# linebender/piet-metal

Measured on AMD Instinct MI355X. Metric: Mpixels/s, Ghostscript Tiger 3840x2160 (fills+strokes): W*H / t_frame, higher is better.
Workload: dtype f32 geometry + f16 accumulators (as the reference)

## Files before the change

### piet_metal_amd/csrc/pm_bin_rows.h

```cpp
#pragma once
#include "pm_kernels_common.h"
#include <pm_params.h>
#include "pm_frame_row.h"

namespace pm {


namespace {

#define PM_PU(field) ParamU32<offsetof(FrameParams, field)>(PR)
#define PM_PP(field) ParamPtr<decltype(FrameParams::field), offsetof(FrameParams, field)>(PR)

}

constexpr uint32_t kCtStride = kStripTiles + 1;
#ifndef PM_BIN_SURV_LDS
#define PM_BIN_SURV_LDS 512
#endif
constexpr uint32_t kSurvLds = PM_BIN_SURV_LDS;
constexpr uint32_t kSupCPL = 2;
constexpr uint32_t kChunkCPL = 4;
static_assert(kSuperChunks == 2 * kChunkCPL && kSupCPL <= kCtStride, "two lanes per surviving super; the list fits in s_ct");
__device__ __forceinline__ float HalfWidthOf(uint32_t aux0) { return 0.5f * __uint_as_float(aux0) + 0.5f; }

// ... 60 lines not shown
    const ParamRegs PR = LoadParams(P);
    const uint32_t tid = threadIdx.x;
    uint4 srd_e = make_uint4(0u, 0u, 0u, 0u);
    if constexpr (kEntry) {
        srd_e = E->sr_desc[blockIdx.x];
        uint2 bb_e = make_uint2(0u, 0u);
        uint32_t it_e = 0;
        if (!E->use_row_lists && tid < E->n_band_items) {
            bb_e = E->band_bbox[tid];
            it_e = E->band_item != nullptr ? E->band_item[tid] : tid;
        }
#pragma unroll
        for (uint32_t u = 0; u < 256u / kBinThreads; ++u)
            L.s_lut[tid + u * kBinThreads] = E->lut_srgb2lin[tid + u * kBinThreads] | (E->lut_unorm2h[tid + u * kBinThreads] << 16);
        L.s_ct[tid] = bb_e.x;
        L.s_ct[kBinThreads + tid] = bb_e.y;
        L.s_ct[2 * kBinThreads + tid] = it_e;
        srd_e = Scalar4(srd_e);
    }
    const bool bin_wt = kOne || PM_PU(bin_wt) != 0u;
    auto put_quad = [&](uint4 *q, const uint4 v) {
        if (bin_wt) StoreWT16(q, v);
        else *q = v;
    };
    const uint32_t lane = LaneId();
    const uint32_t wave = kW == 1 ? 0u : tid >> 6;
    if (blockIdx.x == 0) {
        for (uint32_t k = tid; k < kTicketParts; k += kBinThreads) PM_PP(ctr_next)->ticket[k].count = 0;
        for (uint32_t k = tid; k < kFifos; k += kBinThreads) {
            PM_PP(ctr_next)->fifo[k].tail = 0;
            PM_PP(ctr_next)->fifo[k].head = 0;
        }
        for (uint32_t k = tid; k < kFifoShards; k += kBinThreads) PM_PP(ctr_next)->done_part[k].count = 0;
    }
    if (blockIdx.x == 0 && tid == 0) {
#pragma unroll
        for (uint32_t k = 0; k < kArenaShards; ++k) {
            PM_PP(ctr_next)->ptcl[k].top = 0;
            PM_PP(ctr_next)->ptcl[k].bin_dwords = 0;
        }
#pragma unroll
        for (uint32_t k = 0; k < kClasses; ++k) PM_PP(ctr_next)->cls[k].count = 0;
        PM_PP(ctr_next)->overflow = 0;
        PM_PP(ctr_next)->done_top.parts = 0;
        PM_PP(ctr_next)->done_top.done = 0;
    }
    for (uint32_t rix = blockIdx.x, rix_next = 0; rix < PM_PU(n_sr_active); rix = rix_next) {
    if (rix != blockIdx.x) LdsBarrier();
    const bool first_row = kEntry && rix == blockIdx.x;
    uint4 srd = srd_e;
    if (!first_row) srd = PM_PP(sr_desc)[rix];
    uint32_t n_band = PM_PU(n_band_items);
    const uint2 *band_bbox = PM_PP(band_bbox);
    const uint32_t *band_item = PM_PP(band_item);
    uint2 bb_next = make_uint2(0u, 0u);
    uint32_t it_next = 0;
    if (PM_PU(use_row_lists)) {
        const uint2 srl = PM_PP(sr_list)[rix];
        const uint32_t lo = __builtin_amdgcn_readfirstlane(srl.x);
        n_band = __builtin_amdgcn_readfirstlane(srl.y);
        band_bbox = PM_PP(row_bbox) + lo;
        band_item = PM_PP(row_item) + lo;
    }
    if (first_row && !PM_PU(use_row_lists)) {
        bb_next = make_uint2(L.s_ct[tid], L.s_ct[kBinThreads + tid]);
        it_next = L.s_ct[2 * kBinThreads + tid];
    } else if (tid < n_band) {
        bb_next = band_bbox[tid];
        it_next = band_item != nullptr ? band_item[tid] : tid;
    }
    if constexpr (kOne) rix_next = __builtin_amdgcn_readfirstlane(PM_PP(sr_next_one)[rix]);
    else rix_next = PM_PU(bin_no_chains) ? 0u : __builtin_amdgcn_readfirstlane(srd.w);
    if (rix_next == 0) rix_next = 0xffffffffu;
    const bool last_row = rix_next == 0xffffffffu;
    auto one_keep = [&](uint32_t n_heavy, uint32_t n_queued) -> uint32_t { return last_row ? OneLaunchKeep(n_heavy, n_queued) : 0u; };
    uint32_t lut_word[256 / kBinThreads] = {};
    if constexpr (!kEntry) {
#pragma unroll
        for (uint32_t u = 0; u < 256u / kBinThreads; ++u) lut_word[u] = PM_PP(lut_srgb2lin)[tid + u * kBinThreads] | (PM_PP(lut_unorm2h)[tid + u * kBinThreads] << 16);
    }
    const uint32_t srx = __builtin_amdgcn_readfirstlane(srd.x);
    const uint32_t strip = srx & 0xffu, row_rel = srx >> 16;
    const uint32_t t_beg = (srx >> 8) & 15u, t_cnt = ((srx >> 12) & 15u) + 1u;
    const uint32_t run_mask = ((1u << t_cnt) - 1u) << t_beg;
    const uint32_t sr = row_rel * PM_PU(strips_x) + strip;
    const uint32_t shard = rix % kArenaShards;
    const uint32_t shard_quads = PM_PU(tarena_cap) / kArenaShards;
    const uint32_t shard_base = shard * shard_quads;
    const uint32_t ty = PM_PU(row0) + row_rel;
    const int sx0 = static_cast<int>(strip * kGroupW);
    const int y0 = static_cast<int>(ty * kTileH);
    const int sy0 = y0 & ~static_cast<int>(kGroupH - 1);
    auto uniform_f = [](int v) { return __uint_as_float(static_cast<uint32_t>(__builtin_amdgcn_readfirstlane(static_cast<int>(__float_as_uint(static_cast<float>(v)))))); };
    const float fsx0 = uniform_f(sx0 + static_cast<int>(t_beg * kTileW)), fsx1 = uniform_f(sx0 + static_cast<int>((t_beg + t_cnt) * kTileW));
    const float fstrip0 = uniform_f(sx0), fstrip1 = uniform_f(sx0 + static_cast<int>(kGroupW));
    const float fy0 = uniform_f(y0), fy1 = uniform_f(y0 + static_cast<int>(kTileH));
    const float fsy0 = uniform_f(sy0), fsy1 = uniform_f(sy0 + static_cast<int>(kGroupH));

    auto stamp = [&](uint32_t k) {
        if (kProfile) {
            if constexpr (kProfile) {
                if (tid == 0) L.s_stamp[k] = static_cast<uint32_t>(wall_clock64());
            }
        }
    };
    bool prof_first = true;
    uint32_t prof_chunks = 0;
    if constexpr (kProfile) {
        if (tid < 14) L.s_stamp[tid] = 0;
    }
    stamp(0);
    if (tid < kStripTiles) {
        L.s_est[tid] = 0;
        L.s_last_kept[tid] = 0;
        L.s_last_solid[tid] = 0;
        L.s_solid_rgba[tid] = 0;
        L.s_head_q[tid] = 0;
        L.s_head_n[tid] = 0;
        L.s_prev_q[tid] = 0;
    }
    if (tid == 0) L.s_alloc[1] = 0;
// ... 34 lines not shown
        const uint32_t heavy_classes = PM_PU(split_mode) ? PM_PU(n_heavy_classes) : 0u;
        ForClasses([&](auto kc) {
            constexpr uint32_t k = decltype(kc)::value;
            const uint32_t mk = static_cast<uint32_t>(__ballot(is_queued && cls == k));
            if (cls == k) my_mask = mk;
            if constexpr (kOne) {
                const uint32_t nk = static_cast<uint32_t>(__popc(mk));
                if (cls > k) before += nk;
                if (k < heavy_classes) n_heavy += nk;
                n_queued += nk;
            } else {
                WriteLane<k>(lane_cnt, static_cast<uint32_t>(__popc(mk)));
            }
        });
        const uint32_t slots = is_queued ? ((3u * est + 1u) * kCmdQuadsNum + kCmdQuadsDen - 1u) / kCmdQuadsDen : 0u;
        const uint32_t slots_incl = WaveInclusiveScan(slots);
        TailState ts;
        ts.qtotal = WaveLast(slots_incl);
        ts.list_off = slots_incl - slots;
        ts.packed = (is_queued ? 1u : 0u) | (cls << 1) | (static_cast<uint32_t>(__popc(my_mask & ((1u << Opaque(lane)) - 1u))) << 4);
        ts.pos = before + (ts.packed >> 4);
        ts.n_heavy = n_heavy;
        ts.n_queued = n_queued;
        ts.qres = 0;
        if (ts.qtotal) {
            if constexpr (kOne) {
                const uint32_t n_keep = one_keep(n_heavy, n_queued);
                const uint32_t give_heavy = n_heavy - (n_heavy ? n_keep : 0u);
                const uint32_t give_light = n_queued - n_heavy - (n_heavy ? 0u : n_keep);
                const uint32_t give = lane == 0u ? give_heavy : give_light;
                Fifo *const ff = &PM_PP(ctr_cur)->fifo[lane == 0u ? 0u : 1u + (blockIdx.x & (kFifoShards - 1u))];
                if (lane < 2u && give) ts.qres = atomicAdd(&ff->tail, give);
            } else {
                if (lane < kClasses && lane_cnt) ts.qres = atomicAdd(&PM_PP(ctr_cur)->cls[lane].count, lane_cnt);
            }
            if (lane == kClasses) ts.qres = AtomicAddOneLane(&PM_PP(ctr_cur)->ptcl[shard].top, ts.qtotal);
        }
        const uint32_t tile = row_rel * PM_PU(tiles_x) + strip * kStripTiles + Opaque(lane);
        const uint32_t state = is_queued ? 0u : (is_solid ? L.s_solid_rgba[tl] : 0xffffffffu);
        if constexpr (!kOne) {
            if (lane < kStripTiles) L.s_solid_rgba[tl] = tile_lane ? state : 0u;
        }
        if (tile_lane) {
            if (bin_wt) StoreWT4(PM_PP(tile_state) + tile, state);
            else PM_PP(tile_state)[tile] = state;
        }
        if constexpr (kOne) {
            if (last_row) {
                if (lane < kStripTiles) R->state[tl] = tile_lane ? state : 0u;
                if (lane == 0u) R->striprow = sr;
            } else {
                const uint32_t st = static_cast<uint32_t>(__shfl(static_cast<int>(tile_lane ? state : 0u), static_cast<int>(lane >> 2)));
                const uint32_t px = strip * kGroupW + lane * 4u;
                if (st != 0u && px < PM_PU(width)) {
                    const uint32_t col = StoreOrder(st, PM_PU(fb_bgra));
                    uint8_t *const base = PM_PP(fb) + static_cast<size_t>(row_rel * kTileH) * PM_PU(fb_stride) + static_cast<size_t>(px) * 4;
                    const uint32_t rows_here = min(kTileH, PM_PU(height) - min(PM_PU(height), ty * kTileH));
                    const bool vec = px + 4u <= PM_PU(width) && PM_PU(fb_vec16) != 0u;
                    for (uint32_t rr = 0; rr < rows_here; ++rr) {
                        uint8_t *dst = base + static_cast<size_t>(rr) * PM_PU(fb_stride);
                        if (vec) *reinterpret_cast<uint4 *>(dst) = make_uint4(col, col, col, col);
                        else
                            for (uint32_t k = 0; k < 4u && px + k < PM_PU(width); ++k) reinterpret_cast<uint32_t *>(dst)[k] = col;
                    }
                }
            }
        }
// ... 8 lines not shown
        }
        if (!ts.qtotal) return;
        const uint32_t cls = (ts.packed >> 1) & 7u;
        const uint32_t used = static_cast<uint32_t>(__builtin_amdgcn_readlane(static_cast<int>(ts.qres), kClasses)) + 1u;
        const uint32_t base = shard_base + used;
        const uint32_t q_base = static_cast<uint32_t>(__shfl(static_cast<int>(ts.qres), static_cast<int>(cls)));
        const bool fits = used + ts.qtotal <= shard_quads && used + ts.qtotal >= used && L.s_alloc[1] == 0u;
        if (!fits && lane == 0) {
            PM_PP(ctr_cur)->overflow = 1;
            *PM_PP(host_overflow) = 1;
        }
        if (ts.packed & 1u) {
            const uint32_t ol = Opaque(lane);
            const uint32_t tile = row_rel * PM_PU(tiles_x) + strip * kStripTiles + ol;
            const uint32_t list_slot = fits ? base + ts.list_off : 0xffffffffu;
            PM_PP(tile_ptcl)[tile] = list_slot;
            uint4 entry = make_uint4((strip * kStripTiles + ol) | (row_rel << 16), list_slot, L.s_head_q[ol], L.s_head_n[ol]);
            if constexpr (kOne) {
                if (!fits) entry.w |= 1u;
                const uint32_t n_keep = one_keep(ts.n_heavy, ts.n_queued);
                const uint32_t h_base = static_cast<uint32_t>(__builtin_amdgcn_readlane(static_cast<int>(ts.qres), 0));
                const uint32_t l_base = static_cast<uint32_t>(__builtin_amdgcn_readlane(static_cast<int>(ts.qres), 1));
                const uint32_t cap = PM_PU(fifo_cap);
                if (ts.pos < n_keep) {
                    R->entry[ts.pos] = entry;
                } else if (ts.pos < ts.n_heavy) {
                    const uint32_t ix = h_base + ts.pos - n_keep;
                    if (ix < cap) StoreWT16(PM_PP(fifo) + ix, entry);
                } else {
                    const uint32_t ix = l_base + ts.pos - (ts.n_heavy ? ts.n_heavy : n_keep);
                    if (ix < cap) StoreWT16(PM_PP(fifo) + static_cast<size_t>(1u + (blockIdx.x & (kFifoShards - 1u))) * cap + ix, entry);
                }
            } else {
                put_quad(PM_PP(queue) + (cls * PM_PU(queue_cap) + q_base + (ts.packed >> 4)), entry);
            }
        }
    };

    uint32_t ncand = 0;
    if (region_end - cursor == PM_PU(sr_empty_dwords)) n_band = 0;
    if constexpr (!kEntry) {
#pragma unroll
        for (uint32_t u = 0; u < 256u / kBinThreads; ++u) L.s_lut[tid + u * kBinThreads] = lut_word[u];
    }
    for (uint32_t ib = 0;; ib += kBatch) {
        const bool more = ib < n_band;
        const uint32_t j = ib + tid;
        bool cand = false;
        uint32_t mask = 0;
        const uint2 bb = bb_next;
        const uint32_t i = it_next;
        if (j + kBatch < n_band) {
            bb_next = band_bbox[j + kBatch];
            it_next = band_item != nullptr ? band_item[j + kBatch] : j + kBatch;
        }
        if (more && tid < kBatch && j < n_band) {
            const int bx = static_cast<int>(bb.x & 0xffffu), by = static_cast<int>(bb.x >> 16);
            const int bz = static_cast<int>(bb.y & 0xffffu), bw = static_cast<int>(bb.y >> 16);
            cand = bz >= sx0 && bx < sx0 + static_cast<int>(kGroupW) && bw >= y0 && by < y0 + static_cast<int>(kTileH);
            if (cand) {
                const int t_lo = (bx > sx0) ? ((bx - sx0) >> 4) : 0;
                int t_hi = (bz - sx0) >> 4;
                if (t_hi > 15) t_hi = 15;
                mask = ((2u << t_hi) - 1u) & ~((1u << t_lo) - 1u) & run_mask;
                cand = mask != 0u;
            }
        }
// ... 669 lines not shown
```

### piet_metal_amd/csrc/pm_coarse.hip

```cpp
#include "pm_kernels_common.h"
#include "pm_coarse_tile.h"

namespace pm {


template <bool kCapture>
__global__ __launch_bounds__(kThreads, PM_COARSE_WPS) void pm_coarse_kernel(FrameParams P) {
    __shared__ CoarseLds s_lds[kWaves];
    CoarseLds &L = s_lds[WaveId()];

    const uint32_t lane = LaneId();
    const uint64_t lanes_below = (1ull << lane) - 1ull;
    uint32_t cls_end[kClasses];
    {
        uint32_t run = 0;
#pragma unroll
        for (uint32_t k = 0; k < kClasses; ++k) {
            run += P.ctr_cur->cls[k].count;
            cls_end[k] = run;
        }
    }
    const uint32_t n_total = cls_end[kClasses - 1];

    const uint32_t wave_global = blockIdx.x * kWaves + (WaveId());
    const uint32_t n_waves = gridDim.x * kWaves;

    for (uint32_t pass = 0; pass * n_waves < n_total; ++pass) {
        const uint32_t slot = pass * n_waves + ((pass & 1u) ? (n_waves - 1u - wave_global) : wave_global);
        if (slot >= n_total) continue;
        uint32_t qix = slot;
#pragma unroll
        for (uint32_t k = 1; k < kClasses; ++k)
            if (slot >= cls_end[k - 1]) qix = k * P.queue_cap + (slot - cls_end[k - 1]);
        const uint4 qe = Scalar4(P.queue[qix]);
        CoarseTile<kCapture>(P, L, qe, lane, lanes_below);
        WaveSync();
    }
}


void LaunchCoarse(const FrameParams &p, uint32_t grid, bool capture, hipStream_t stream, hipEvent_t t0, hipEvent_t t1) {
    if (capture)
        PM_LAUNCH(pm_coarse_kernel<true>, dim3(grid), dim3(kThreads), stream, t0, t1, p);
    else
        PM_LAUNCH(pm_coarse_kernel<false>, dim3(grid), dim3(kThreads), stream, t0, t1, p);
}

}
```

### piet_metal_amd/csrc/pm_context.hip

```cpp
#include <hip/hip_runtime.h>

#include <algorithm>
#include <chrono>
#include <cmath>
#include <cstdio>
#include <cstdlib>
#include <cstring>
#include <new>
#include <string>
#include <vector>

#include "../../include/piet_metal_amd.h"
#include "pm_device.h"
#include "pm_flatten.h"
#include "pm_hit_test.h"
#include "pm_layout.h"

namespace {

thread_local std::string g_last_error;

void SetError(const std::string &s) { g_last_error = s; }

int HipFail(hipError_t e, const char *what) {
// ... 64 lines not shown
            l->lin2srgb[h] = 0;
            continue;
        }
        float y;
        if (x < thr) {
            y = HalfBitsToFloat(RoundHalf(k * x));
        } else {
            const float p = HalfBitsToFloat(HalfBitsFromDouble(std::pow(static_cast<double>(x), ex)));
            const float sp = HalfBitsToFloat(RoundHalf(s * p));
            y = HalfBitsToFloat(RoundHalf(sp - o));
        }
        const float cl = std::fmin(std::fmax(y, 0.0f), 1.0f);
        l->lin2srgb[h] = static_cast<uint8_t>(std::rintf(cl * 255.0f));
    }
}

}


namespace {
constexpr int kMaxSlots = 16;
constexpr int kDefaultFrameStreams = 4;

int EnvInt(const char *name, int dflt, int lo, int hi) {
    const char *v = std::getenv(name);
    if (!v || !*v) return dflt;
    return std::max(lo, std::min(hi, std::atoi(v)));
}
}

struct FrameSlot {
    uint8_t *d_fb = nullptr;
    size_t fb_cap = 0;
    size_t tables_cap = 0;
    uint32_t *d_arena = nullptr;
    uint32_t arena_cap = 0;
    uint4 *d_queue = nullptr;
    uint32_t *d_tile_state = nullptr;
    uint32_t *d_tile_ptcl = nullptr;
    uint32_t *d_tile_ncmd = nullptr;
    uint4 *d_ptcl = nullptr;
    uint32_t ptcl_cap = 0;
    uint2 *d_row_bbox = nullptr;
    uint32_t *d_row_item = nullptr;
    uint64_t row_cap = 0;
    uint32_t state_epoch = 0;
    uint32_t vp_epoch = 0;
    pm::Counters *d_ctr = nullptr;
    uint32_t *h_overflow = nullptr;
    uint32_t *d_overflow = nullptr;
    uint4 *d_fifo = nullptr;
    uint32_t fifo_cap = 0;
    uint32_t parity = 0;
    hipEvent_t ev_done = nullptr;
    bool in_flight = false;
    bool needs_check = false;
    pm::FrameParams params{};
    hipStream_t frame_stream = nullptr;
    bool user_stream = false;
};

struct pm_ctx {
    int device = 0;
    hipStream_t stream = nullptr;
    std::vector<hipStream_t> streams;
    bool fold_clear = true;
// ... 113 lines not shown
    uint32_t query_keep = 0;
    bool idle_seen = false;
    uint32_t query_every = 8;
    int last_slot = -1;

    pm::FlattenCache flatten_cache;
    bool scene_from_paths = false;

    hipEvent_t ev_scene = nullptr;
    hipEvent_t ev_hit = nullptr;
    hipStream_t hit_stream = nullptr;
    bool hit_pending = false;
    uint8_t *d_hit = nullptr;
    size_t hit_cap = 0;

    float t_flatten_ms = 0, t_index_ms = 0, t_arena_ms = 0;
    uint32_t plans_made = 0;

    uint32_t *d_lut_srgb2lin = nullptr;
    uint32_t *d_lut_unorm2h = nullptr;
    uint8_t *d_lut_lin2srgb = nullptr;
};

namespace {

struct WallTimer {
    std::chrono::steady_clock::time_point t0 = std::chrono::steady_clock::now();
    float ms() const { return std::chrono::duration<float, std::milli>(std::chrono::steady_clock::now() - t0).count(); }
};

uint32_t BandRows(const pm_ctx *c) { return c->row1 - c->row0; }
size_t BandTiles(const pm_ctx *c) { return std::max<size_t>(static_cast<size_t>(BandRows(c)) * c->tiles_x, 1); }

int SyncAll(pm_ctx *c) {
    for (hipStream_t q : c->streams) PM_TRY(hipStreamSynchronize(q));
    for (auto &s : c->slot) {
        if (s.in_flight && s.user_stream) PM_TRY(hipEventSynchronize(s.ev_done));
        s.in_flight = false;
    }
    if (c->hit_pending) PM_TRY(hipEventSynchronize(c->ev_hit));
    c->hit_pending = false;
    return PM_OK;
}

void FreeSlotViewport(FrameSlot *s) {
    if (s->d_fb) (void)hipFree(s->d_fb);
    if (s->d_queue) (void)hipFree(s->d_queue);
    if (s->d_fifo) (void)hipFree(s->d_fifo);
    s->d_fifo = nullptr;
    s->fifo_cap = 0;
    s->d_fb = nullptr;
    s->d_queue = nullptr;
    s->fb_cap = s->tables_cap = 0;
    s->d_tile_state = s->d_tile_ptcl = s->d_tile_ncmd = nullptr;
    s->state_epoch = 0;
}

void FreeViewport(pm_ctx *c) {
    for (auto &s : c->slot) {
        FreeSlotViewport(&s);
        s.in_flight = false;
        s.needs_check = false;
    }
    c->last_slot = -1;
}

int AllocSlotViewport(pm_ctx *c, FrameSlot *s) {
    if (s->d_fb && s->vp_epoch == c->vp_epoch) return PM_OK;
    const size_t tiles = BandTiles(c);
    const size_t tables = std::max<size_t>(tiles, 4);
    const size_t fb_want = std::max<size_t>(c->fb_bytes, 16);
    hipError_t e = hipSuccess;
    if (s->d_fb && s->d_queue && s->fb_cap >= fb_want && s->tables_cap >= tables) {
        if (s->d_fifo) (void)hipFree(s->d_fifo);
        s->d_fifo = nullptr;
        s->fifo_cap = 0;
    } else {
        FreeSlotViewport(s);
        e = hipMalloc(&s->d_fb, fb_want);
        if (e == hipSuccess) e = hipMalloc(&s->d_queue, pm::kClasses * tables * sizeof(uint4) + 3 * tables * sizeof(uint32_t));
        if (e == hipSuccess) {
            s->fb_cap = fb_want;
            s->tables_cap = tables;
        }
    }
    s->vp_epoch = c->vp_epoch;
    if (e == hipSuccess) {
        s->d_tile_state = reinterpret_cast<uint32_t *>(s->d_queue + pm::kClasses * tables);
        s->d_tile_ptcl = s->d_tile_state + tables;
        s->d_tile_ncmd = s->d_tile_ptcl + tables;
    }
    s->state_epoch = 0;
    if (e != hipSuccess) {
        if (s->d_fb) (void)hipFree(s->d_fb);
        if (s->d_queue) (void)hipFree(s->d_queue);
        s->d_fb = nullptr;
        s->d_queue = nullptr;
        s->fb_cap = s->tables_cap = 0;
        s->d_tile_state = s->d_tile_ptcl = s->d_tile_ncmd = nullptr;
        return HipFail(e, "hipMalloc(frame slot viewport buffers)");
    }
    return PM_OK;
}

int AllocViewport(pm_ctx *c) {
    c->vp_epoch += 1;
    for (auto &s : c->slot) {
        s.in_flight = false;
        s.needs_check = false;
        if (s.h_overflow) s.h_overflow[2] = 0;
    }
    c->last_slot = -1;
    const uint32_t rows = BandRows(c);
    c->fb_stride = static_cast<size_t>(c->width) * 4;
    c->fb_bytes = c->fb_stride * static_cast<size_t>(rows) * pm::kTileH;
    const int r0 = AllocSlotViewport(c, &c->slot[0]);
    if (r0 != PM_OK) return r0;
    c->arena_dirty = true;
    c->plan_reusable = false;
    c->fb_slots.clear();
    c->fb_applied = false;
    return PM_OK;
}

int ValidateScene(const uint8_t *meta, size_t meta_len, size_t scene_bytes, uint32_t *n_items_out) {
    if (scene_bytes < 8 || meta_len < 8) return PM_ERR_SCENE;
    uint32_t n, items_ix;
    std::memcpy(&n, meta, 4);
    std::memcpy(&items_ix, meta + 4, 4);
    const uint64_t bbox_end = 8ull + 8ull * n;
    const uint64_t items_end = static_cast<uint64_t>(items_ix) + 32ull * n;
// ... 458 lines not shown
    if (r != PM_OK) return r;
    const float t_plan = tm.ms();
    r = EnsureSlotBuffers(c, s);
    if (r != PM_OK) return r;
    if (tm.ms() > 0.05f && std::getenv("PM_HOST_TIMING")) std::fprintf(stderr, "BuildParams: plan %.3f slot buffers %.3f ms (arena %u dwords, tile arena %llu quads)\n", t_plan, tm.ms() - t_plan, c->arena_cap, static_cast<unsigned long long>(c->ptcl_want));
    if (!fb) fb = s->d_fb;
    std::memset(p, 0, sizeof(*p));
    p->scene = c->d_scene;
    p->scene_bytes = static_cast<uint32_t>(c->scene_bytes);
    p->n_items = c->n_items;
    p->items_ix = c->dev_items_ix;
    p->bbox_ix = c->dev_bbox_ix;
    p->width = c->width;
    p->height = c->height;
    p->tiles_x = c->tiles_x;
    p->tiles_y = c->tiles_y;
    p->row0 = c->row0;
    p->row1 = c->row1;
    p->strips_x = c->strips_x;
    p->fb = fb;
    p->fb_stride = static_cast<uint32_t>(stride);
    p->fb_vec16 = ((reinterpret_cast<uintptr_t>(fb) & 15u) == 0 && (stride & 15u) == 0) ? 1u : 0u;
    p->fb_bgra = c->target_fmt == PM_FMT_BGRA8 ? 1u : 0u;
    p->arena = s->d_arena;
    p->arena_cap = s->arena_cap;
    p->sr_desc = c->d_sr_desc;
    p->sr_list = c->d_sr_list;
    p->n_sr_active = c->n_sr_active;
    p->sr_slots = c->d_sr_slots;
    p->bin_prio_slots = c->bin_prio_slots;
    p->bin_grid = c->bin_grid;
    p->sr_empty_dwords = c->sr_empty_dwords;
    p->queue = s->d_queue;
    p->queue_cap = static_cast<uint32_t>(BandTiles(c));
    p->tile_state = s->d_tile_state;
    p->tarena = s->d_ptcl;
    p->tarena_cap = s->ptcl_cap;
    p->tile_ptcl = s->d_tile_ptcl;
    p->tile_ncmd = s->d_tile_ncmd;
    p->ctr_cur = s->d_ctr + s->parity;
    p->ctr_next = s->d_ctr + (s->parity ^ 1u);
    p->host_overflow = s->d_overflow;
    p->host_fail = s->d_overflow + 1;
    p->host_dense = s->d_overflow + 2;
    p->fine_dense = 0;
    p->fifo = s->d_fifo;
    p->fifo_cap = s->fifo_cap;
    p->one_launch = 0;
    p->sr_next_one = c->d_sr_next_one;
    p->one_grid_rows = c->one_grid_rows;
    p->idle_sr = c->d_idle_sr;
    p->n_idle_sr = c->n_idle_sr;
    p->spin_ticks = c->frame_spin_ticks;
    p->band_bbox = c->band_identity ? reinterpret_cast<const uint2 *>(c->d_scene + c->dev_bbox_ix) : c->d_band_bbox;
    p->band_item = c->band_identity ? nullptr : c->d_band_item;
    p->n_band_items = c->n_band_items;
    p->bin_waves = c->bin_waves;
    p->clear_in_bin = c->fold_clear_mode == 4 || (c->fold_clear_mode == 3 && c->n_sr_active > c->bin_grid) ? 1u : 0u;
    p->bin_wt = c->bin_wt_mode == 1 || (c->bin_wt_mode == 2 && c->n_sr_active <= c->bin_grid) ? 1u : 0u;
    p->split_mode = c->split_mode;
    p->dense_factor = c->dense_factor;
    p->verdict_waves = static_cast<uint32_t>(c->n_cus) * c->fine_wg_per_cu * 4u;
    {
        SetClassThresholds(c, p, c->heavy_stream_lone);
        p->n_heavy_classes = 3;
        p->handout_static = c->handout == 1 ? 1u : 0u;
    }
// ... 637 lines not shown
    delete l;
    if (e != hipSuccess) return fail(e, "lookup tables");
    if (EnvInt("PM_PREALLOC", 1, 0, 1)) {
        e = c->flatten_cache.Reserve(4096, 65536);
        if (e == hipSuccess) e = hipMalloc(&c->d_chunk_base, (65536 + 1) * sizeof(uint32_t));
        if (e == hipSuccess) c->chunk_base_cap = 65536 + 1;
        if (e == hipSuccess) e = hipMalloc(&c->d_chunk_bbox, (1u << 19) * sizeof(float4));
        if (e == hipSuccess) c->chunk_bbox_cap = 1u << 19;
        if (e == hipSuccess) e = hipMalloc(&c->d_sup_bbox, (1u << 16) * sizeof(float4));
        if (e == hipSuccess) c->sup_bbox_cap = 1u << 16;
        if (e == hipSuccess) e = hipMalloc(&c->d_sr_desc, 65536 * sizeof(uint4));
        if (e == hipSuccess) e = hipMalloc(&c->d_sr_list, 65536 * sizeof(uint2));
        if (e == hipSuccess) e = hipMalloc(&c->d_sr_slots, 65536 * sizeof(uint32_t));
        if (e == hipSuccess) e = hipMalloc(&c->d_sr_desc_whole, 65536 * sizeof(uint4));
        if (e == hipSuccess) c->sr_desc_cap = 65536;
        if (e == hipSuccess) e = hipMalloc(&c->d_band_bbox, 65536 * sizeof(uint2));
        if (e == hipSuccess) e = hipMalloc(&c->d_band_item, 65536 * sizeof(uint32_t));
        if (e == hipSuccess) c->band_cap = 65536;
#ifdef PM_EMU
        const int arena_mb = 192, tile_mb = 96, slots_dflt = 1;
#else
        const int arena_mb = 2304, tile_mb = 1792, slots_dflt = static_cast<int>(kMaxSlots);
#endif
        const size_t n_pre = std::min<size_t>(c->slot.size(), static_cast<size_t>(EnvInt("PM_PREALLOC_SLOTS", slots_dflt, 1, static_cast<int>(kMaxSlots))));
        const size_t px = static_cast<size_t>(EnvInt("PM_PREALLOC_MPIXELS", 64, 0, 4096)) << 20;
        const size_t tables = std::max<size_t>(px / (pm::kTileW * pm::kTileH), 4);
        const uint32_t arena0 = static_cast<uint32_t>(EnvInt("PM_PREALLOC_ARENA_MB", arena_mb, 1, 12288)) << 18;
        const uint32_t tile0 = std::max<uint32_t>(static_cast<uint32_t>(EnvInt("PM_PREALLOC_TILE_MB", tile_mb, 1, 16384)) << 16,
                                                  ((1u << 22) * pm::kCmdQuadsNum) / pm::kCmdQuadsDen);
        for (size_t si = 0; si < n_pre && e == hipSuccess; ++si) {
            FrameSlot &fs = c->slot[si];
            if (px != 0) {
                e = hipMalloc(&fs.d_fb, px * 4);
                if (e == hipSuccess) e = hipMalloc(&fs.d_queue, pm::kClasses * tables * sizeof(uint4) + 3 * tables * sizeof(uint32_t));
                if (e == hipSuccess) {
                    fs.fb_cap = px * 4;
                    fs.tables_cap = tables;
                }
            }
            if (e == hipSuccess) e = hipMalloc(&fs.d_arena, static_cast<size_t>(arena0) * sizeof(uint32_t));
            if (e == hipSuccess) fs.arena_cap = arena0;
            if (e == hipSuccess && !std::getenv("PM_PTCL_INITIAL_CMDS")) {
                e = hipMalloc(&fs.d_ptcl, static_cast<size_t>(tile0) * sizeof(uint4));
                if (e == hipSuccess) fs.ptcl_cap = tile0;
            }
        }
        if (e != hipSuccess) return fail(e, "working-set reservation");
    }
    if (ReserveScene(c, 16u << 20) != PM_OK) {
        *err = PM_ERR_HIP;
        pm_destroy(c);
        return nullptr;
    }
    if (EnvInt("PM_WARMUP", 1, 0, 1)) {
        const pm_path wp = {0u, 3u, PM_PATH_FILL | PM_PATH_STROKE, 0x000000ffu, 0x000000ffu, 1.0f};
        pm_path_el we[3] = {};
        we[0].tag = PM_EL_MOVE; we[0].p[0] = 2.0; we[0].p[1] = 2.0;
        we[1].tag = PM_EL_LINE; we[1].p[0] = 12.0; we[1].p[1] = 3.0;
        we[2].tag = PM_EL_CURVE; we[2].p[0] = 12.0; we[2].p[1] = 8.0; we[2].p[2] = 8.0; we[2].p[3] = 12.0; we[2].p[4] = 3.0; we[2].p[5] = 12.0;
        const double ident[6] = {1.0, 0.0, 0.0, 1.0, 0.0, 0.0};
        int rw = pm_resize(c, 40, 24);
        if (rw == PM_OK) rw = pm_flatten_and_encode(c, &wp, 1, we, 3, ident, 1.0f, nullptr, nullptr);
        if (rw == PM_OK) rw = pm_render(c);
        if (rw == PM_OK) rw = pm_sync(c);
        if (rw != PM_OK) {
            *err = rw;
            pm_destroy(c);
            return nullptr;
        }
        InvalidateScene(c);
// ... 710 lines not shown
        else if (ok)
            ok = hipEventElapsedTime(&v[1], tev[1], tev[4]) == hipSuccess && hipEventElapsedTime(&v[2], tev[4], tev[5]) == hipSuccess &&
                 hipEventElapsedTime(&v[3], tev[5], tev[6]) == hipSuccess;
        if (ok)
            for (int k = 0; k < 6; ++k) col[k].push_back(v[k]);
    }
    for (auto &v : tev)
        if (v) (void)hipEventDestroy(v);
    if (r != PM_OK) return r;
    if (col[0].empty()) return PM_ERR_HIP;
    for (int k = 0; k < 6; ++k) {
        std::sort(col[k].begin(), col[k].end());
        out6[k] = col[k][col[k].size() / 2];
    }
    return pm_sync(c);
}

int pm_get_stats(pm_ctx *c, pm_stats *out) {
    if (!c || !out) return PM_ERR_INVALID;
    std::memset(out, 0, sizeof(*out));
    PM_TRY(hipSetDevice(c->device));
    int r = SyncAll(c);
    if (r != PM_OK) return r;
    out->tiles_x = c->tiles_x;
    out->tiles_y = c->tiles_y;
    out->band_row0 = c->row0;
    out->band_row1 = c->row1;
    out->n_items = c->n_items;
    out->arena_cap_dwords = c->arena_cap;
    out->scene_bytes = static_cast<uint32_t>(c->user_scene_bytes);
    if (c->last_slot >= 0) {
        pm::Counters k;
        PM_TRY(hipMemcpy(&k, c->slot[c->last_slot].params.ctr_cur, sizeof(k), hipMemcpyDeviceToHost));
        for (uint32_t q = 0; q < pm::kClasses; ++q) out->queued_tiles += k.cls[q].count;
        for (uint32_t q = 0; q < 3; ++q) out->heavy_tiles += k.cls[q].count;
        out->arena_used_dwords = 0;
        for (uint32_t i = 0; i < pm::kArenaShards; ++i) out->arena_used_dwords += k.ptcl[i].bin_dwords;
        out->ptcl_used_cmds = 0;
        for (uint32_t i = 0; i < pm::kArenaShards; ++i) out->ptcl_used_cmds += k.ptcl[i].top;
        out->overflow = k.overflow;
    }
    return PM_OK;
}

int pm_get_scene_timings(pm_ctx *c, pm_scene_timings *out) {
    if (!c || !out) return PM_ERR_INVALID;
    out->flatten_encode_ms = c->t_flatten_ms;
    out->scene_index_ms = c->t_index_ms;
    out->arena_setup_ms = c->t_arena_ms;
    return PM_OK;
}

int pm_get_binning_plans(pm_ctx *c, uint32_t *plans) {
    if (!c || !plans) return PM_ERR_INVALID;
    *plans = c->plans_made;
    return PM_OK;
}

int pm_fill_coverage(pm_ctx *c, uint32_t item_ix, float *dst, size_t dst_stride_floats) {
    if (!c || !dst || dst_stride_floats < c->width) return PM_ERR_INVALID;
    PM_TRY(hipSetDevice(c->device));
    int r = pm_sync(c);
    if (r != PM_OK) return r;
    if (c->scene_bytes < 8 || item_ix >= c->n_items || c->tiles_x == 0) {
        SetError("pm_fill_coverage: no such item (or no scene / viewport)");
        return PM_ERR_INVALID;
    }
    const uint8_t *meta = c->item_meta.data();
// ... 275 lines not shown
    PM_TRY(hipMalloc(&d, std::max<size_t>(rows, 1) * 16 * sizeof(unsigned long long)));
    PM_TRY(hipMemset(d, 0, std::max<size_t>(rows, 1) * 16 * sizeof(unsigned long long)));
    const int si = static_cast<int>(c->frame % c->slot.size());
    FrameSlot *s = &c->slot[si];
    pm::FrameParams p;
    r = BuildParams(c, s, nullptr, c->fb_stride, &p);
    if (r == PM_OK) {
        p.dbg_bin = d;
        hipError_t e = ResetTileState(c, s, c->stream);
        pm::LaunchBin(p, c->stream);
        if (!c->fold_clear && !p.clear_in_bin) pm::LaunchClear(p, BandRows(c) * c->strips_x, c->stream);
        if (!c->fused) pm::LaunchCoarse(p, CoarseGrid(c), false, c->stream);
        pm::LaunchFine(p, c->fold_clear && !p.clear_in_bin ? BandRows(c) * c->strips_x : 0u, c->fused, c->stream);
        p.dbg_bin = nullptr;
        Submitted(c, si, p, c->stream);
        if (e == hipSuccess) e = hipStreamSynchronize(c->stream);
        if (e == hipSuccess) e = hipMemcpy(out, d, rows * 16 * sizeof(unsigned long long), hipMemcpyDeviceToHost);
        if (e != hipSuccess) r = HipFail(e, "bin timeline");
    }
    (void)hipFree(d);
    return r;
}

int pm_debug_time_tiles(pm_ctx *c, uint64_t *out, size_t max_slots, size_t *n_slots) {
    if (!c || !out || c->last_slot < 0) return PM_ERR_INVALID;
    PM_TRY(hipSetDevice(c->device));
    int r = pm_sync(c);
    if (r != PM_OK) return r;
    FrameSlot *s = &c->slot[c->last_slot];
    pm::Counters k;
    PM_TRY(hipMemcpy(&k, s->params.ctr_cur, sizeof(k), hipMemcpyDeviceToHost));
    size_t heavy = 0, total = 0;
    for (uint32_t q = 0; q < pm::kClasses; ++q) {
        total += k.cls[q].count;
        if (q < 3) heavy += k.cls[q].count;
    }
    const bool dense = heavy * c->dense_factor >= static_cast<size_t>(s->params.fine_grid) * 4u || c->split_mode == 0;
    const size_t slots = dense ? total : 4 * heavy + (total - heavy);
    if (n_slots) *n_slots = slots;
    if (slots > max_slots) return PM_ERR_CAPACITY;
    unsigned long long *d = nullptr;
    PM_TRY(hipMalloc(&d, std::max<size_t>(slots, 1) * 12 * sizeof(unsigned long long)));
    pm::FrameParams p = s->params;
    p.dbg_time = d;
    PM_TRY(hipMemsetAsync(&p.ctr_cur->ticket, 0, sizeof(p.ctr_cur->ticket), c->stream));
    pm::LaunchFine(p, 0u, c->fused, c->stream);
    hipError_t e = hipStreamSynchronize(c->stream);
    if (e == hipSuccess) e = hipMemcpy(out, d, slots * 12 * sizeof(unsigned long long), hipMemcpyDeviceToHost);
    (void)hipFree(d);
    if (e != hipSuccess) return HipFail(e, "tile timeline");
    return PM_OK;
}

void init_test_scene(uint8_t *buf, ssize_t buf_size) {
    if (!buf || buf_size <= 0) {
        SetError("init_test_scene: bad buffer");
        return;
    }
    int err = PM_OK;
    pm_ctx *c = pm_create(0, &err);
    if (!c) return;
    pm_svg *svg = pm_svg_tiger(0, &err);
    if (svg) {
        const double scale = 8.0;
        const double affine[6] = {scale, 0.0, 0.0, scale, 0.0, 0.0};
        size_t bytes = 0;
        uint32_t items = 0;
        err = pm_flatten_and_encode(c, pm_svg_paths(svg), pm_svg_n_paths(svg), pm_svg_els(svg), pm_svg_n_els(svg), affine,
// ... 12 lines not shown
```

### piet_metal_amd/csrc/pm_device.h

```cpp
#pragma once

#include <hip/hip_runtime.h>

#include <cstdint>

#include "pm_layout.h"

namespace pm {

constexpr uint32_t kClasses = 8;

constexpr uint32_t kTicketParts = 32;

constexpr uint32_t kArenaShards = 16;
constexpr uint32_t kFifoShards = 8;
constexpr uint32_t kFifos = 1 + kFifoShards;

struct Fifo {
    uint32_t tail;
    uint32_t head;
    uint32_t pad[30];
};

struct Counters {
    struct {
        uint32_t top;
        uint32_t bin_dwords;
        uint32_t pad[30];
    } ptcl[kArenaShards];
    struct {
        uint32_t count;
        uint32_t pad[31];
    } cls[kClasses];
    uint32_t overflow;
    uint32_t pad4[31];
    struct {
        uint32_t count;
        uint32_t pad[31];
    } ticket[kTicketParts];
    Fifo fifo[kFifos];
    struct {
        uint32_t count;
        uint32_t pad[31];
    } done_part[kFifoShards];
    struct {
        uint32_t parts;
        uint32_t done;
        uint32_t pad[30];
    } done_top;
};

constexpr uint32_t kChunkSegs = 4;
constexpr uint32_t kSuperChunks = 8;
constexpr uint32_t kArenaBase = 4;
constexpr int kBinWaves = 4;
constexpr uint32_t kRowCullPer = 8;
constexpr uint32_t kRowCullStep = 64u * kBinWaves * kRowCullPer;
constexpr uint32_t kCtShift = 20;
constexpr uint32_t kCtCountMask = (1u << kCtShift) - 1u;
constexpr uint32_t kSlotDwords = 5;
constexpr uint32_t kPieceHitBits = 9;
constexpr uint32_t kPieceHitMask = (1u << kPieceHitBits) - 1u;
constexpr uint32_t kCmdQuadsNum = 3, kCmdQuadsDen = 2;

struct FrameParams {
    const uint8_t *scene;
    uint32_t scene_bytes;
    uint32_t n_items, items_ix;
    uint32_t bbox_ix;
    uint32_t width, height;
    uint32_t tiles_x, tiles_y;
    uint32_t row0, row1;
    uint32_t strips_x;
    uint8_t *fb;
    uint32_t fb_stride;
    uint32_t fb_vec16;
    uint32_t fb_bgra;
    uint32_t *arena;
    uint32_t arena_cap;
    const uint4 *sr_desc;
    const uint2 *sr_list;
    uint32_t n_sr_active;
    uint32_t *sr_slots;
    uint32_t bin_grid;
    uint32_t bin_prio_slots;
    uint32_t sr_empty_dwords;
    uint4 *queue;
    uint32_t queue_cap;
    uint32_t *tile_state;
    uint4 *tarena;
    uint32_t tarena_cap;
    uint32_t *tile_ptcl;
    uint32_t *tile_ncmd;
    Counters *ctr_cur;
    Counters *ctr_next;
    uint32_t *host_overflow;
    const uint2 *band_bbox;
    const uint32_t *band_item;
    uint32_t n_band_items;
    uint32_t bin_waves;
    uint32_t fine_grid;
    uint32_t split_mode;
    uint32_t fine_dense;
    uint32_t *host_dense;
    uint32_t verdict_waves;
    uint32_t dense_factor;
    uint32_t class_thr[kClasses - 1];
    uint32_t n_heavy_classes;
    uint32_t handout_static;
    uint32_t use_row_lists;
    const uint32_t *row_base;
    uint32_t bin_no_chains;
    uint32_t clear_in_bin;
    uint32_t bin_wt;
    uint32_t row_parts;
    uint32_t row_part_items;
    uint2 *row_bbox;
    uint32_t *row_item;
    const uint32_t *chunk_base;
    const float4 *chunk_bbox;
    const float4 *sup_bbox;
// ... 33 lines not shown
```

### piet_metal_amd/csrc/pm_fine.hip

```cpp
#include "pm_fine_tile.h"
#include <type_traits>

namespace pm {

__global__ __launch_bounds__(kBinThreads) void pm_clear_kernel(FrameParams P) { ClearStripRow(P, blockIdx.x); }

template <bool kFused, bool kProf, bool kCapture = false, bool kDense = false>
__global__ __launch_bounds__(kThreads, kDense ? 6 : 5) void pm_fine_kernel(FrameParams P) {
    __shared__ std::conditional_t<kDense, DenseLds, SparseLds> S;
    if (blockIdx.x >= P.fine_grid) {
        ClearStripRow(P, blockIdx.x - P.fine_grid);
        return;
    }
    const uint32_t lane = LaneId(), wave = WaveId();
    uint32_t cls_end[kClasses];
    {
        uint32_t run = 0;
#pragma unroll
        for (uint32_t k = 0; k < kClasses; ++k) {
            run += P.ctr_cur->cls[k].count;
            cls_end[k] = run;
        }
    }
    uint32_t wg = blockIdx.x;
    if ((P.fine_grid & 31u) == 0u) {
        const uint32_t xcd = wg & 7u, i = wg >> 3;
        wg = (((i >> 2) << 3) + xcd) * 4u + (i & 3u);
    }
    const uint32_t wave_global = wg * kWaves + wave;
    const uint32_t n_waves = P.fine_grid * kWaves;
    const uint32_t n_tiles = cls_end[kClasses - 1];
    const uint32_t n_heavy = P.n_heavy_classes ? cls_end[min(P.n_heavy_classes, kClasses) - 1u] : 0u;
    const bool dense = kDense || static_cast<uint64_t>(n_heavy) * P.dense_factor >= n_waves || P.split_mode == 0;
    if (blockIdx.x == 0 && threadIdx.x == 0 && P.host_dense != nullptr)
        *P.host_dense = (static_cast<uint64_t>(n_heavy) * P.dense_factor >= P.verdict_waves || P.split_mode == 0 || n_heavy == 0u) ? 2u : 1u;
    const uint32_t sh = dense ? 0u : 2u;
    const uint32_t s_h = n_heavy << sh;
    const uint32_t n_slots = s_h + (n_tiles - n_heavy);
    auto slot_entry = [&](uint32_t slot) -> uint32_t {
        const uint32_t t = slot < s_h ? (slot >> sh) : n_heavy + (slot - s_h);
        uint32_t qix = t;
#pragma unroll
        for (uint32_t k = 1; k < kClasses; ++k)
            if (t >= cls_end[k - 1]) qix = k * P.queue_cap + (t - cls_end[k - 1]);
        return qix;
    };
    auto pass_slot = [&](uint32_t pass) -> uint32_t {
        return pass * n_waves + ((pass & 1u) ? (n_waves - 1u - wave_global) : wave_global);
    };
    const uint64_t lanes_below = (1ull << lane) - 1ull;
    const uint32_t static_passes = P.handout_static ? 0x7fffffffu / n_waves : (dense ? 1u : max(1u, (s_h + n_waves - 1u) / n_waves));
    const uint32_t n_static = static_passes * n_waves;
    const uint32_t n_decks = min(kTicketParts, n_waves);
    const uint32_t part = wave_global % n_decks;
    uint32_t *const deck_ctr = &P.ctr_cur->ticket[part].count;
    uint32_t slot = pass_slot(0);
    uint4 qe = make_uint4(0u, 0u, 0u, 0u);
    uint32_t qix = 0;
    bool have = slot < n_slots;
    if (have) {
        qix = slot_entry(slot);
        qe = P.queue[qix];
    }
    for (uint32_t pass = 0; have; ++pass) {
        const uint32_t cur_slot = slot;
        const uint4 cur = Scalar4(qe);
        const bool draws = pass + 1u >= static_passes;
        if (!draws) {
            slot = pass_slot(pass + 1u);
            have = slot < n_slots;
            if (have) {
                qix = slot_entry(slot);
                qe = P.queue[qix];
            }
        }
        auto next_card = [&]() {
            if (!draws) return;
            uint32_t j = 0;
// ... 118 lines not shown
```

### piet_metal_amd/csrc/pm_kernels_common.h

```cpp
#pragma once

#include <hip/hip_runtime.h>
#include <hip/hip_ext.h>

#include <cstddef>
#include <utility>

#include "pm_device.h"
#include <pm_pin.h>

namespace pm {

namespace {

#ifndef PM_COARSE_WPS
#define PM_COARSE_WPS 5
#endif
#ifndef PM_FINE_WPS
#define PM_FINE_WPS 5
#endif
constexpr int kThreads = 256;
constexpr int kWaves = kThreads / 64;
constexpr int kBinThreads = 64 * kBinWaves;
constexpr uint32_t kBatch = 256;
// ... 13 lines not shown
                                     __builtin_amdgcn_mbcnt_lo(static_cast<uint32_t>(mask), 0u));
}

__device__ __forceinline__ uint32_t WaveInclusiveScan(uint32_t v) {
    int x = static_cast<int>(v);
    x += __builtin_amdgcn_update_dpp(0, x, 0x111, 0xf, 0xf, false);
    x += __builtin_amdgcn_update_dpp(0, x, 0x112, 0xf, 0xf, false);
    x += __builtin_amdgcn_update_dpp(0, x, 0x114, 0xf, 0xf, false);
    x += __builtin_amdgcn_update_dpp(0, x, 0x118, 0xf, 0xf, false);
    x += __builtin_amdgcn_update_dpp(0, x, 0x142, 0xa, 0xf, false);
    x += __builtin_amdgcn_update_dpp(0, x, 0x143, 0xc, 0xf, false);
    return static_cast<uint32_t>(x);
}

__device__ __forceinline__ uint32_t WaveInclusiveMax(uint32_t v) {
    int x = static_cast<int>(v);
    auto mx = [](int a, int b) { return static_cast<int>(max(static_cast<uint32_t>(a), static_cast<uint32_t>(b))); };
    x = mx(x, __builtin_amdgcn_update_dpp(0, x, 0x111, 0xf, 0xf, false));
    x = mx(x, __builtin_amdgcn_update_dpp(0, x, 0x112, 0xf, 0xf, false));
    x = mx(x, __builtin_amdgcn_update_dpp(0, x, 0x114, 0xf, 0xf, false));
    x = mx(x, __builtin_amdgcn_update_dpp(0, x, 0x118, 0xf, 0xf, false));
    x = mx(x, __builtin_amdgcn_update_dpp(0, x, 0x142, 0xa, 0xf, false));
    x = mx(x, __builtin_amdgcn_update_dpp(0, x, 0x143, 0xc, 0xf, false));
    return static_cast<uint32_t>(x);
}

__device__ __forceinline__ uint32_t WaveAtHighest(uint32_t v, uint64_t mask) {
    const int l = __builtin_amdgcn_readfirstlane(63 - __builtin_clzll(mask));
    return static_cast<uint32_t>(__builtin_amdgcn_readlane(static_cast<int>(v), l));
}

__device__ __forceinline__ uint32_t WaveLast(uint32_t v) {
    return static_cast<uint32_t>(__builtin_amdgcn_readlane(static_cast<int>(v), 63));
}

__device__ __forceinline__ void WaveSync() { __builtin_amdgcn_fence(__ATOMIC_ACQ_REL, "wavefront"); __builtin_amdgcn_wave_barrier(); }

__device__ __forceinline__ void LdsBarrier() {
#ifdef PM_STRICT_BARRIERS
    __syncthreads();
#else
    __builtin_amdgcn_fence(__ATOMIC_RELEASE, "workgroup", "local");
    __builtin_amdgcn_s_barrier();
    __builtin_amdgcn_fence(__ATOMIC_ACQUIRE, "workgroup", "local");
#endif
}

__device__ __forceinline__ float Sgn(float x) { return (x > 0.0f) ? 1.0f : ((x < 0.0f) ? -1.0f : 0.0f); }
__device__ __forceinline__ float Sat(float x) { return fminf(fmaxf(x, 0.0f), 1.0f); }

__device__ __forceinline__ bool Straddles(float s00, float s01, float s10, float s11) {
    return s00 * s01 + s00 * s10 + s00 * s11 < 3.0f;
}

__device__ __forceinline__ uint32_t StoreOrder(uint32_t rgba, uint32_t bgra) {
    return bgra ? ((rgba & 0xff00ff00u) | ((rgba & 0xffu) << 16) | ((rgba >> 16) & 0xffu)) : rgba;
}

#ifndef PM_FB_WT
#define PM_FB_WT 1
#endif
__device__ __forceinline__ void StorePixels4(uint8_t *dst, uint4 v) {
#if PM_FB_WT
    StoreWT16(reinterpret_cast<uint4 *>(dst), v);
#else
    *reinterpret_cast<uint4 *>(dst) = v;
// ... 240 lines not shown
```

Baseline: 172,400.

## Shard per-class tile queue counters across eight cursors to cut atomic contention

Each tile class now has eight counters (one per shard, chosen by row index), and each shard gets its own queue sub-region, so binning blocks spread their atomicAdds across 64 cursors instead of hammering 8. Coarse and fine kernels rebuild the slot-to-queue mapping with a wave-wide prefix scan over the 64 cursors and a ballot lookup, replacing the serial per-class loop. Queue allocation and capacity checks are resized to cover the sharded sub-caps. The cost is a larger queue footprint, an extra LDS round trip with two barriers in the fine kernel, and tile order within a class that now interleaves by shard.

```diff
diff --git a/piet_metal_amd/csrc/pm_bin_rows.h b/piet_metal_amd/csrc/pm_bin_rows.h
--- a/piet_metal_amd/csrc/pm_bin_rows.h
+++ b/piet_metal_amd/csrc/pm_bin_rows.h
@@ -116,6 +116,7 @@
             PM_PP(ctr_next)->fifo[k].head = 0;
         }
         for (uint32_t k = tid; k < kFifoShards; k += kBinThreads) PM_PP(ctr_next)->done_part[k].count = 0;
+        for (uint32_t k = tid; k < kClassCursors; k += kBinThreads) PM_PP(ctr_next)->cls[k % kClassShards].count[k / kClassShards] = 0;
     }
     if (blockIdx.x == 0 && tid == 0) {
 #pragma unroll
@@ -123,8 +124,6 @@
             PM_PP(ctr_next)->ptcl[k].top = 0;
             PM_PP(ctr_next)->ptcl[k].bin_dwords = 0;
         }
-#pragma unroll
-        for (uint32_t k = 0; k < kClasses; ++k) PM_PP(ctr_next)->cls[k].count = 0;
         PM_PP(ctr_next)->overflow = 0;
         PM_PP(ctr_next)->done_top.parts = 0;
         PM_PP(ctr_next)->done_top.done = 0;
@@ -171,6 +170,7 @@
     const uint32_t shard = rix % kArenaShards;
     const uint32_t shard_quads = PM_PU(tarena_cap) / kArenaShards;
     const uint32_t shard_base = shard * shard_quads;
+    const uint32_t cls_shard = rix % kClassShards;
     const uint32_t ty = PM_PU(row0) + row_rel;
     const int sx0 = static_cast<int>(strip * kGroupW);
     const int y0 = static_cast<int>(ty * kTileH);
@@ -271,7 +271,7 @@
                 Fifo *const ff = &PM_PP(ctr_cur)->fifo[lane == 0u ? 0u : 1u + (blockIdx.x & (kFifoShards - 1u))];
                 if (lane < 2u && give) ts.qres = atomicAdd(&ff->tail, give);
             } else {
-                if (lane < kClasses && lane_cnt) ts.qres = atomicAdd(&PM_PP(ctr_cur)->cls[lane].count, lane_cnt);
+                if (lane < kClasses && lane_cnt) ts.qres = atomicAdd(&PM_PP(ctr_cur)->cls[cls_shard].count[lane], lane_cnt);
             }
             if (lane == kClasses) ts.qres = AtomicAddOneLane(&PM_PP(ctr_cur)->ptcl[shard].top, ts.qtotal);
         }
@@ -346,7 +346,7 @@
                     if (ix < cap) StoreWT16(PM_PP(fifo) + static_cast<size_t>(1u + (blockIdx.x & (kFifoShards - 1u))) * cap + ix, entry);
                 }
             } else {
-                put_quad(PM_PP(queue) + (cls * PM_PU(queue_cap) + q_base + (ts.packed >> 4)), entry);
+                put_quad(PM_PP(queue) + ((cls * kClassShards + cls_shard) * PM_PU(queue_sub_cap) + q_base + (ts.packed >> 4)), entry);
             }
         }
     };
diff --git a/piet_metal_amd/csrc/pm_coarse.hip b/piet_metal_amd/csrc/pm_coarse.hip
--- a/piet_metal_amd/csrc/pm_coarse.hip
+++ b/piet_metal_amd/csrc/pm_coarse.hip
@@ -11,16 +11,8 @@
 
     const uint32_t lane = LaneId();
     const uint64_t lanes_below = (1ull << lane) - 1ull;
-    uint32_t cls_end[kClasses];
-    {
-        uint32_t run = 0;
-#pragma unroll
-        for (uint32_t k = 0; k < kClasses; ++k) {
-            run += P.ctr_cur->cls[k].count;
-            cls_end[k] = run;
-        }
-    }
-    const uint32_t n_total = cls_end[kClasses - 1];
+    const uint32_t q_prefix = ClassQueuePrefix(P.ctr_cur, lane);
+    const uint32_t n_total = WaveLast(q_prefix);
 
     const uint32_t wave_global = blockIdx.x * kWaves + (WaveId());
     const uint32_t n_waves = gridDim.x * kWaves;
@@ -28,11 +20,7 @@
     for (uint32_t pass = 0; pass * n_waves < n_total; ++pass) {
         const uint32_t slot = pass * n_waves + ((pass & 1u) ? (n_waves - 1u - wave_global) : wave_global);
         if (slot >= n_total) continue;
-        uint32_t qix = slot;
-#pragma unroll
-        for (uint32_t k = 1; k < kClasses; ++k)
-            if (slot >= cls_end[k - 1]) qix = k * P.queue_cap + (slot - cls_end[k - 1]);
-        const uint4 qe = Scalar4(P.queue[qix]);
+        const uint4 qe = Scalar4(P.queue[ClassQueueEntry(q_prefix, slot, P.queue_sub_cap)]);
         CoarseTile<kCapture>(P, L, qe, lane, lanes_below);
         WaveSync();
     }
diff --git a/piet_metal_amd/csrc/pm_context.hip b/piet_metal_amd/csrc/pm_context.hip
--- a/piet_metal_amd/csrc/pm_context.hip
+++ b/piet_metal_amd/csrc/pm_context.hip
@@ -120,6 +120,7 @@
 struct FrameSlot {
     uint8_t *d_fb = nullptr;
     size_t fb_cap = 0;
+    size_t queue_cap = 0;
     size_t tables_cap = 0;
     uint32_t *d_arena = nullptr;
     uint32_t arena_cap = 0;
@@ -299,6 +300,11 @@
 uint32_t BandRows(const pm_ctx *c) { return c->row1 - c->row0; }
 size_t BandTiles(const pm_ctx *c) { return std::max<size_t>(static_cast<size_t>(BandRows(c)) * c->tiles_x, 1); }
 
+size_t QueueSubCap(size_t tiles, size_t entries) {
+    return std::min<size_t>(std::max<size_t>(tiles, 1), pm::kStripTiles * ((std::max<size_t>(entries, 1) + pm::kClassShards - 1) / pm::kClassShards));
+}
+size_t QueueEntries(size_t tiles, size_t strip_rows) { return std::max<size_t>(pm::kClassCursors * QueueSubCap(tiles, 2 * strip_rows), 4); }
+
 int SyncAll(pm_ctx *c) {
     for (hipStream_t q : c->streams) PM_TRY(hipStreamSynchronize(q));
     for (auto &s : c->slot) {
@@ -318,7 +324,7 @@
     s->fifo_cap = 0;
     s->d_fb = nullptr;
     s->d_queue = nullptr;
-    s->fb_cap = s->tables_cap = 0;
+    s->fb_cap = s->tables_cap = s->queue_cap = 0;
     s->d_tile_state = s->d_tile_ptcl = s->d_tile_ncmd = nullptr;
     s->state_epoch = 0;
 }
@@ -336,24 +342,26 @@
     if (s->d_fb && s->vp_epoch == c->vp_epoch) return PM_OK;
     const size_t tiles = BandTiles(c);
     const size_t tables = std::max<size_t>(tiles, 4);
+    const size_t queue_want = QueueEntries(tiles, static_cast<size_t>(BandRows(c)) * c->strips_x);
     const size_t fb_want = std::max<size_t>(c->fb_bytes, 16);
     hipError_t e = hipSuccess;
-    if (s->d_fb && s->d_queue && s->fb_cap >= fb_want && s->tables_cap >= tables) {
+    if (s->d_fb && s->d_queue && s->fb_cap >= fb_want && s->tables_cap >= tables && s->queue_cap >= queue_want) {
         if (s->d_fifo) (void)hipFree(s->d_fifo);
         s->d_fifo = nullptr;
         s->fifo_cap = 0;
     } else {
         FreeSlotViewport(s);
         e = hipMalloc(&s->d_fb, fb_want);
-        if (e == hipSuccess) e = hipMalloc(&s->d_queue, pm::kClasses * tables * sizeof(uint4) + 3 * tables * sizeof(uint32_t));
+        if (e == hipSuccess) e = hipMalloc(&s->d_queue, queue_want * sizeof(uint4) + 3 * tables * sizeof(uint32_t));
         if (e == hipSuccess) {
             s->fb_cap = fb_want;
             s->tables_cap = tables;
+            s->queue_cap = queue_want;
         }
     }
     s->vp_epoch = c->vp_epoch;
     if (e == hipSuccess) {
-        s->d_tile_state = reinterpret_cast<uint32_t *>(s->d_queue + pm::kClasses * tables);
+        s->d_tile_state = reinterpret_cast<uint32_t *>(s->d_queue + s->queue_cap);
         s->d_tile_ptcl = s->d_tile_state + tables;
         s->d_tile_ncmd = s->d_tile_ptcl + tables;
     }
@@ -363,7 +371,7 @@
         if (s->d_queue) (void)hipFree(s->d_queue);
         s->d_fb = nullptr;
         s->d_queue = nullptr;
-        s->fb_cap = s->tables_cap = 0;
+        s->fb_cap = s->tables_cap = s->queue_cap = 0;
         s->d_tile_state = s->d_tile_ptcl = s->d_tile_ncmd = nullptr;
         return HipFail(e, "hipMalloc(frame slot viewport buffers)");
     }
@@ -888,7 +896,11 @@
     p->bin_grid = c->bin_grid;
     p->sr_empty_dwords = c->sr_empty_dwords;
     p->queue = s->d_queue;
-    p->queue_cap = static_cast<uint32_t>(BandTiles(c));
+    p->queue_sub_cap = static_cast<uint32_t>(QueueSubCap(BandTiles(c), std::max(c->n_sr_active, c->n_sr_whole)));
+    if (static_cast<size_t>(pm::kClassCursors) * p->queue_sub_cap > s->queue_cap) {
+        SetError("the work list is longer than the slot's tile queues were sized for");
+        return PM_ERR_CAPACITY;
+    }
     p->tile_state = s->d_tile_state;
     p->tarena = s->d_ptcl;
     p->tarena_cap = s->ptcl_cap;
@@ -1592,10 +1604,12 @@
             FrameSlot &fs = c->slot[si];
             if (px != 0) {
                 e = hipMalloc(&fs.d_fb, px * 4);
-                if (e == hipSuccess) e = hipMalloc(&fs.d_queue, pm::kClasses * tables * sizeof(uint4) + 3 * tables * sizeof(uint32_t));
+                const size_t queue_pre = QueueEntries(tables, tables / pm::kStripTiles);
+                if (e == hipSuccess) e = hipMalloc(&fs.d_queue, queue_pre * sizeof(uint4) + 3 * tables * sizeof(uint32_t));
                 if (e == hipSuccess) {
                     fs.fb_cap = px * 4;
                     fs.tables_cap = tables;
+                    fs.queue_cap = queue_pre;
                 }
             }
             if (e == hipSuccess) e = hipMalloc(&fs.d_arena, static_cast<size_t>(arena0) * sizeof(uint32_t));
@@ -2372,8 +2386,12 @@
     if (c->last_slot >= 0) {
         pm::Counters k;
         PM_TRY(hipMemcpy(&k, c->slot[c->last_slot].params.ctr_cur, sizeof(k), hipMemcpyDeviceToHost));
-        for (uint32_t q = 0; q < pm::kClasses; ++q) out->queued_tiles += k.cls[q].count;
-        for (uint32_t q = 0; q < 3; ++q) out->heavy_tiles += k.cls[q].count;
+        for (uint32_t q = 0; q < pm::kClasses; ++q) {
+            for (uint32_t sh = 0; sh < pm::kClassShards; ++sh) {
+                out->queued_tiles += k.cls[sh].count[q];
+                if (q < 3) out->heavy_tiles += k.cls[sh].count[q];
+            }
+        }
         out->arena_used_dwords = 0;
         for (uint32_t i = 0; i < pm::kArenaShards; ++i) out->arena_used_dwords += k.ptcl[i].bin_dwords;
         out->ptcl_used_cmds = 0;
@@ -2715,8 +2733,10 @@
     PM_TRY(hipMemcpy(&k, s->params.ctr_cur, sizeof(k), hipMemcpyDeviceToHost));
     size_t heavy = 0, total = 0;
     for (uint32_t q = 0; q < pm::kClasses; ++q) {
-        total += k.cls[q].count;
-        if (q < 3) heavy += k.cls[q].count;
+        for (uint32_t sh = 0; sh < pm::kClassShards; ++sh) {
+            total += k.cls[sh].count[q];
+            if (q < 3) heavy += k.cls[sh].count[q];
+        }
     }
     const bool dense = heavy * c->dense_factor >= static_cast<size_t>(s->params.fine_grid) * 4u || c->split_mode == 0;
     const size_t slots = dense ? total : 4 * heavy + (total - heavy);
diff --git a/piet_metal_amd/csrc/pm_device.h b/piet_metal_amd/csrc/pm_device.h
--- a/piet_metal_amd/csrc/pm_device.h
+++ b/piet_metal_amd/csrc/pm_device.h
@@ -9,6 +9,9 @@
 namespace pm {
 
 constexpr uint32_t kClasses = 8;
+constexpr uint32_t kClassShards = 8;
+constexpr uint32_t kClassCursors = kClasses * kClassShards;
+static_assert(kClassCursors == 64, "a cursor per lane");
 
 constexpr uint32_t kTicketParts = 32;
 
@@ -29,9 +32,9 @@
         uint32_t pad[30];
     } ptcl[kArenaShards];
     struct {
-        uint32_t count;
-        uint32_t pad[31];
-    } cls[kClasses];
+        uint32_t count[kClasses];
+        uint32_t pad[32 - kClasses];
+    } cls[kClassShards];
     uint32_t overflow;
     uint32_t pad4[31];
     struct {
@@ -86,7 +89,7 @@
     uint32_t bin_prio_slots;
     uint32_t sr_empty_dwords;
     uint4 *queue;
-    uint32_t queue_cap;
+    uint32_t queue_sub_cap;
     uint32_t *tile_state;
     uint4 *tarena;
     uint32_t tarena_cap;
diff --git a/piet_metal_amd/csrc/pm_fine.hip b/piet_metal_amd/csrc/pm_fine.hip
--- a/piet_metal_amd/csrc/pm_fine.hip
+++ b/piet_metal_amd/csrc/pm_fine.hip
@@ -13,15 +13,12 @@
         return;
     }
     const uint32_t lane = LaneId(), wave = WaveId();
-    uint32_t cls_end[kClasses];
-    {
-        uint32_t run = 0;
-#pragma unroll
-        for (uint32_t k = 0; k < kClasses; ++k) {
-            run += P.ctr_cur->cls[k].count;
-            cls_end[k] = run;
-        }
-    }
+    uint32_t *const q_share = reinterpret_cast<uint32_t *>(S.w[0].cmds);
+    static_assert(sizeof(S.w[0].cmds) >= kClassCursors * sizeof(uint32_t), "the sums fit wave 0's staging area");
+    if (wave == 0) q_share[lane] = ClassQueuePrefix(P.ctr_cur, lane);
+    LdsBarrier();
+    const uint32_t q_prefix = q_share[lane];
+    LdsBarrier();
     uint32_t wg = blockIdx.x;
     if ((P.fine_grid & 31u) == 0u) {
         const uint32_t xcd = wg & 7u, i = wg >> 3;
@@ -29,8 +26,8 @@
     }
     const uint32_t wave_global = wg * kWaves + wave;
     const uint32_t n_waves = P.fine_grid * kWaves;
-    const uint32_t n_tiles = cls_end[kClasses - 1];
-    const uint32_t n_heavy = P.n_heavy_classes ? cls_end[min(P.n_heavy_classes, kClasses) - 1u] : 0u;
+    const uint32_t n_tiles = WaveLast(q_prefix);
+    const uint32_t n_heavy = P.n_heavy_classes ? ClassQueueTotal(q_prefix, min(P.n_heavy_classes, kClasses)) : 0u;
     const bool dense = kDense || static_cast<uint64_t>(n_heavy) * P.dense_factor >= n_waves || P.split_mode == 0;
     if (blockIdx.x == 0 && threadIdx.x == 0 && P.host_dense != nullptr)
         *P.host_dense = (static_cast<uint64_t>(n_heavy) * P.dense_factor >= P.verdict_waves || P.split_mode == 0 || n_heavy == 0u) ? 2u : 1u;
@@ -39,11 +36,7 @@
     const uint32_t n_slots = s_h + (n_tiles - n_heavy);
     auto slot_entry = [&](uint32_t slot) -> uint32_t {
         const uint32_t t = slot < s_h ? (slot >> sh) : n_heavy + (slot - s_h);
-        uint32_t qix = t;
-#pragma unroll
-        for (uint32_t k = 1; k < kClasses; ++k)
-            if (t >= cls_end[k - 1]) qix = k * P.queue_cap + (t - cls_end[k - 1]);
-        return qix;
+        return ClassQueueEntry(q_prefix, t, P.queue_sub_cap);
     };
     auto pass_slot = [&](uint32_t pass) -> uint32_t {
         return pass * n_waves + ((pass & 1u) ? (n_waves - 1u - wave_global) : wave_global);
diff --git a/piet_metal_amd/csrc/pm_kernels_common.h b/piet_metal_amd/csrc/pm_kernels_common.h
--- a/piet_metal_amd/csrc/pm_kernels_common.h
+++ b/piet_metal_amd/csrc/pm_kernels_common.h
@@ -69,6 +69,18 @@
 
 __device__ __forceinline__ uint32_t WaveLast(uint32_t v) {
     return static_cast<uint32_t>(__builtin_amdgcn_readlane(static_cast<int>(v), 63));
+}
+
+__device__ __forceinline__ uint32_t ClassQueuePrefix(const Counters *ctr, uint32_t lane) {
+    return WaveInclusiveScan(ctr->cls[lane % kClassShards].count[lane / kClassShards]);
+}
+__device__ __forceinline__ uint32_t ClassQueueTotal(uint32_t prefix, uint32_t n_classes) {
+    return static_cast<uint32_t>(__builtin_amdgcn_readlane(static_cast<int>(prefix), static_cast<int>(n_classes * kClassShards - 1u)));
+}
+__device__ __forceinline__ uint32_t ClassQueueEntry(uint32_t prefix, uint32_t t, uint32_t queue_sub_cap) {
+    const uint32_t owner = static_cast<uint32_t>(__builtin_amdgcn_readfirstlane(static_cast<int>(__builtin_ctzll(__ballot(prefix > t) | (1ull << 63)))));
+    const uint32_t below = static_cast<uint32_t>(__builtin_amdgcn_readlane(static_cast<int>(prefix), static_cast<int>(owner ? owner - 1u : 0u)));
+    return owner * queue_sub_cap + (t - (owner ? below : 0u));
 }
 
 __device__ __forceinline__ void WaveSync() { __builtin_amdgcn_fence(__ATOMIC_ACQ_REL, "wavefront"); __builtin_amdgcn_wave_barrier(); }
```

After: 181,900 (median of 6 runs). 5.5% higher.
